# audioku/meta-transfer-learning

Measured on AMD Instinct MI355X. Metric: meta-steps/sec, higher is better.
Workload: dtype f32 (emulated: 3x3 conv + input Linear on 2 x fp16 pieces "h2" = 22 significand bits, big GEMMs and attention (d_k = 64) on 3 x bf16 pieces "x3" = exact fp32 operands, small products on fp32 MFMA, element-wise on VALU; fp32 accumulation everywhere)

## Files before the change

meta-transfer-learning_amd/csrc/mtl_mfma.hip:

```cpp
#include <cstdlib>
#include <type_traits>

#include "mtl_common.h"
#include "mtl_h2.h"
#include "../../include/mtl_hip.h"

namespace {

constexpr int BK = 32;
constexpr int NT = 256;

template <int ROWS>
struct LdsK {
    static constexpr int LD = BK + 1;
    static constexpr int SIZE = ROWS * LD;
    static __device__ __forceinline__ int at(int row, int k) { return row * LD + k; }
};
template <int ROWS>
struct LdsMN {
    static constexpr int LD = ROWS + 4;
    static constexpr int SIZE = BK * LD;
    static __device__ __forceinline__ int at(int row, int k) { return k * LD + row; }
};

// ... 534 lines not shown
struct EpiConvDgrad {
    float* dx;
    const float* act;
    int b, t0, f0, T, F, Cout, n0;
    __device__ __forceinline__ void store4(int lr, int lc, const float (&v)[4]) const {
        const int col = n0 + lc;
        const int w = (lr >> 5) * 8 + ((lr >> 2) & 7);
#pragma unroll
        for (int j = 0; j < 4; ++j) {
            const int t = t0 + 2 * (w >> 3) + (j & 1), f = f0 + 2 * (w & 7) + (j >> 1);
            if (t < T && f < F) {
                const long o = (((long)b * T + t) * F + f) * Cout + col;
                dx[o] = act[o] > 0.f ? v[j] : 0.f;
            }
        }
    }
    __device__ __forceinline__ void gate4(int lr, int lc, float (&m)[4]) const {
        const int col = n0 + lc;
        const int w = (lr >> 5) * 8 + ((lr >> 2) & 7);
#pragma unroll
        for (int j = 0; j < 4; ++j) {
            const int t = min(t0 + 2 * (w >> 3) + (j & 1), T - 1), f = min(f0 + 2 * (w & 7) + (j >> 1), F - 1);
            m[j] = __builtin_nontemporal_load(act + (((long)b * T + t) * F + f) * Cout + col);
        }
    }
    __device__ __forceinline__ void store4g(int lr, int lc, const float (&v)[4], const float (&m)[4]) const {
        const int col = n0 + lc;
        const int w = (lr >> 5) * 8 + ((lr >> 2) & 7);
#pragma unroll
        for (int j = 0; j < 4; ++j) {
            const int t = t0 + 2 * (w >> 3) + (j & 1), f = f0 + 2 * (w & 7) + (j >> 1);
            if (t < T && f < F) __builtin_nontemporal_store(m[j] > 0.f ? v[j] : 0.f, dx + (((long)b * T + t) * F + f) * Cout + col);
        }
    }
    __device__ __forceinline__ void gate4x2(int lr, int lc, f32x2v (&m)[4]) const {
        const int col = n0 + lc;
        const int w = (lr >> 5) * 8 + ((lr >> 2) & 7);
#pragma unroll
        for (int j = 0; j < 4; ++j) {
            const int t = min(t0 + 2 * (w >> 3) + (j & 1), T - 1), f = min(f0 + 2 * (w & 7) + (j >> 1), F - 1);
            m[j] = __builtin_nontemporal_load(reinterpret_cast<const f32x2v*>(act + (((long)b * T + t) * F + f) * Cout + col));
        }
    }
    __device__ __forceinline__ void store4x2g(int lr, int lc, const float (&v0)[4], const float (&v1)[4], const f32x2v (&m)[4]) const {
        const int col = n0 + lc;
        const int w = (lr >> 5) * 8 + ((lr >> 2) & 7);
#pragma unroll
        for (int j = 0; j < 4; ++j) {
            const int t = t0 + 2 * (w >> 3) + (j & 1), f = f0 + 2 * (w & 7) + (j >> 1);
            const f32x2v o = {m[j].x > 0.f ? v0[j] : 0.f, m[j].y > 0.f ? v1[j] : 0.f};
            if (t < T && f < F) __builtin_nontemporal_store(o, reinterpret_cast<f32x2v*>(dx + (((long)b * T + t) * F + f) * Cout + col));
        }
    }
};

struct ConvP {
    const float* x;
    const uint8_t* am_in;
    const float* w;
    const float* bias;
    const float* act;
    float* y;
    uint8_t* am_out;
    ConvGeom g;
    int ntile;
};

enum { EPI_RELU = 0, EPI_POOL = 1, EPI_DGRAD = 2 };

template <int BN, bool UNPOOL, int EPI>
__global__ __launch_bounds__(NT) void conv3x3_kernel(ConvP p) {
    using LA = LoadConvA<UNPOOL>;
    using LB = LoadMNMajor<BN, true>;
    using E = Engine<128, BN, LA, LB>;
    extern __shared__ __attribute__((aligned(16))) float smem[];
    const int tid = threadIdx.x;
    const int b = blockIdx.z / p.ntile, n0 = (blockIdx.z % p.ntile) * BN;
    const int t0 = blockIdx.y * 8, f0 = blockIdx.x * 16;
    LA la;
    LB lb;
    la.init(p.x, p.am_in, p.g, p.g.Cin, b, t0, f0, tid);
    lb.init(p.w, p.g.Cout, n0, p.g.Cout, 9 * p.g.Cin, tid);
    f32x16 acc[E::TM][E::TN];
    E::zero(acc);
    E::run(la, lb, 9 * p.g.Cin / BK, smem, acc);
    if (EPI == EPI_RELU) {
        EpiConvRelu e{p.y, p.bias, b, t0, f0, p.g.T, p.g.F, p.g.Cout, n0};
        E::finish(acc, e);
    } else if (EPI == EPI_POOL) {
        EpiConvPool e{p.y, p.am_out, p.bias, b, t0, f0, p.g.Tp, p.g.Fp, p.g.Cout, n0};
        E::finish(acc, e);
    } else {
        EpiConvDgrad e{p.y, p.act, b, t0, f0, p.g.T, p.g.F, p.g.Cout, n0};
        E::finish(acc, e);
    }
}

template <int BN, bool UNPOOL, int EPI>
int launch_conv(const ConvP& p, int Te, int Fe, hipStream_t s) {
    using E = Engine<128, BN, LoadConvA<UNPOOL>, LoadMNMajor<BN, true>>;
    static int attr = set_smem(conv3x3_kernel<BN, UNPOOL, EPI>, E::SMEM_BYTES);
    if (attr) return attr;
    dim3 grid((Fe + 15) / 16, (Te + 7) / 8, p.g.B * p.ntile);
    hipLaunchKernelGGL((conv3x3_kernel<BN, UNPOOL, EPI>), grid, dim3(NT), E::SMEM_BYTES, s, p);
    MTL_CHECK_LAUNCH();
    return MTL_OK;
}

template <bool UNPOOL, int EPI>
int dispatch_conv(ConvP& p, int Te, int Fe, hipStream_t s) {
    if (p.g.Cin % 32 || p.g.Cout % 64) return MTL_EINVAL;
    if (p.g.Cout % 128 == 0) {
        p.ntile = p.g.Cout / 128;
        return launch_conv<128, UNPOOL, EPI>(p, Te, Fe, s);
    }
    p.ntile = p.g.Cout / 64;
    return launch_conv<64, UNPOOL, EPI>(p, Te, Fe, s);
}

typedef __bf16 bf16x8 __attribute__((ext_vector_type(8)));
typedef __bf16 bf16x4 __attribute__((ext_vector_type(4)));
constexpr int X3_ROWB = 80;

__device__ __forceinline__ void split3(float x, __bf16& h, __bf16& m, __bf16& l) {
    h = (__bf16)x;
    const float r = x - (float)h;
    m = (__bf16)r;
    l = (__bf16)(r - (float)m);
}

typedef __bf16 bf16x2 __attribute__((ext_vector_type(2)));
__device__ __forceinline__ void split3x2(float x0, float x1, unsigned& h, unsigned& m, unsigned& l) {
    h = __builtin_bit_cast(unsigned, __builtin_convertvector(f32x2{x0, x1}, bf16x2));
    const float r0 = x0 - __builtin_bit_cast(float, h << 16), r1 = x1 - __builtin_bit_cast(float, h & 0xffff0000u);
    m = __builtin_bit_cast(unsigned, __builtin_convertvector(f32x2{r0, r1}, bf16x2));
    const float q0 = r0 - __builtin_bit_cast(float, m << 16), q1 = r1 - __builtin_bit_cast(float, m & 0xffff0000u);
    l = __builtin_bit_cast(unsigned, __builtin_convertvector(f32x2{q0, q1}, bf16x2));
}
__device__ __forceinline__ void split3x4(const float4& v, bf16x4& h, bf16x4& m, bf16x4& l) {
    uint2 hh, mm, ll;
    split3x2(v.x, v.y, hh.x, mm.x, ll.x);
    split3x2(v.z, v.w, hh.y, mm.y, ll.y);
    h = __builtin_bit_cast(bf16x4, hh);
    m = __builtin_bit_cast(bf16x4, mm);
    l = __builtin_bit_cast(bf16x4, ll);
}

typedef float f32x4 __attribute__((ext_vector_type(4)));
#ifndef X3H_IH
#define X3H_IH 0
#endif
#ifndef X3H_M16
#define X3H_M16 1
#endif
template <int NP>
struct Split;
template <>
struct Split<3> {
    static __device__ __forceinline__ void x2(float x0, float x1, float, unsigned (&pc)[3]) { split3x2(x0, x1, pc[0], pc[1], pc[2]); }
    static __device__ __forceinline__ f32x16 mfma(const uint4 (&a)[3], const uint4 (&b)[3], f32x16 cc) {
        const bf16x8 a0 = __builtin_bit_cast(bf16x8, a[0]), a1 = __builtin_bit_cast(bf16x8, a[1]), a2 = __builtin_bit_cast(bf16x8, a[2]);
        const bf16x8 b0 = __builtin_bit_cast(bf16x8, b[0]), b1 = __builtin_bit_cast(bf16x8, b[1]), b2 = __builtin_bit_cast(bf16x8, b[2]);
        cc = __builtin_amdgcn_mfma_f32_32x32x16_bf16(a2, b0, cc, 0, 0, 0);
        cc = __builtin_amdgcn_mfma_f32_32x32x16_bf16(a1, b1, cc, 0, 0, 0);
        cc = __builtin_amdgcn_mfma_f32_32x32x16_bf16(a0, b2, cc, 0, 0, 0);
        cc = __builtin_amdgcn_mfma_f32_32x32x16_bf16(a1, b0, cc, 0, 0, 0);
        cc = __builtin_amdgcn_mfma_f32_32x32x16_bf16(a0, b1, cc, 0, 0, 0);
        return __builtin_amdgcn_mfma_f32_32x32x16_bf16(a0, b0, cc, 0, 0, 0);
    }
    static __device__ __forceinline__ f32x4 mfma16(const uint4 (&a)[3], const uint4 (&b)[3], f32x4 cc) {
        const bf16x8 a0 = __builtin_bit_cast(bf16x8, a[0]), a1 = __builtin_bit_cast(bf16x8, a[1]), a2 = __builtin_bit_cast(bf16x8, a[2]);
        const bf16x8 b0 = __builtin_bit_cast(bf16x8, b[0]), b1 = __builtin_bit_cast(bf16x8, b[1]), b2 = __builtin_bit_cast(bf16x8, b[2]);
        cc = __builtin_amdgcn_mfma_f32_16x16x32_bf16(a2, b0, cc, 0, 0, 0);
        cc = __builtin_amdgcn_mfma_f32_16x16x32_bf16(a1, b1, cc, 0, 0, 0);
        cc = __builtin_amdgcn_mfma_f32_16x16x32_bf16(a0, b2, cc, 0, 0, 0);
        cc = __builtin_amdgcn_mfma_f32_16x16x32_bf16(a1, b0, cc, 0, 0, 0);
        cc = __builtin_amdgcn_mfma_f32_16x16x32_bf16(a0, b1, cc, 0, 0, 0);
        return __builtin_amdgcn_mfma_f32_16x16x32_bf16(a0, b0, cc, 0, 0, 0);
    }
};
template <>
struct Split<2> {
    static __device__ __forceinline__ void x2(float x0, float x1, float s, unsigned (&pc)[2]) { split2x2(x0 * s, x1 * s, pc[0], pc[1]); }
    static __device__ __forceinline__ f32x16 mfma(const uint4 (&a)[2], const uint4 (&b)[2], f32x16 cc) { return h2_mfma(a, b, cc); }
    static __device__ __forceinline__ f32x4 mfma16(const uint4 (&a)[2], const uint4 (&b)[2], f32x4 cc) {
        const f16x8 a0 = __builtin_bit_cast(f16x8, a[0]), a1 = __builtin_bit_cast(f16x8, a[1]);
        const f16x8 b0 = __builtin_bit_cast(f16x8, b[0]), b1 = __builtin_bit_cast(f16x8, b[1]);
        cc = __builtin_amdgcn_mfma_f32_16x16x32_f16(a1, b0, cc, 0, 0, 0);
        cc = __builtin_amdgcn_mfma_f32_16x16x32_f16(a0, b1, cc, 0, 0, 0);
        return __builtin_amdgcn_mfma_f32_16x16x32_f16(a0, b0, cc, 0, 0, 0);
    }
};
template <int NP>
__device__ __forceinline__ void split_x4(const float4& v, float s, uint2 (&pc)[NP]) {
    unsigned a[NP], b[NP];
    Split<NP>::x2(v.x, v.y, s, a);
    Split<NP>::x2(v.z, v.w, s, b);
#pragma unroll
    for (int q = 0; q < NP; ++q) pc[q] = make_uint2(a[q], b[q]);
}


constexpr int WSCALE_PARTS = 16;
template <int NP>
__global__ void conv_wprep_x3_kernel(const float* w, unsigned short* wf, unsigned short* wd, int Cout, int Cin) {
    const int total = 9 * Cin * Cout;
    const int nkf = 9 * (Cin / 32), nkd = 9 * (Cout / 32);
    float s = 1.f;
    if (NP == 2) {
        float* hf = reinterpret_cast<float*>(wf + (long)NP * total);
        float mx = 0.f;
#pragma unroll
        for (int i = 1; i <= WSCALE_PARTS; ++i) mx = fmaxf(mx, hf[i]);
        s = pow2_scale(mx);
        if (blockIdx.x == 0 && threadIdx.x == 0) {
            hf[0] = s;
            *reinterpret_cast<float*>(wd + (long)NP * total) = s;
        }
    }
    for (int e = blockIdx.x * blockDim.x + threadIdx.x; e < total; e += gridDim.x * blockDim.x) {
        const int tap = e % 9;
        const int cin = (e / 9) % Cin;
        const int cout = e / (9 * Cin);
        unsigned pc[NP];
        Split<NP>::x2(w[e], 0.f, s, pc);
#pragma unroll
        for (int p = 0; p < NP; ++p) {
            const unsigned short v = (unsigned short)(pc[p] & 0xffffu);
            wf[(((long)p * nkf + tap * (Cin / 32) + (cin >> 5)) * Cout + cout) * 32 + x3_swz(cin & 31, cout)] = v;
            wd[(((long)p * nkd + (8 - tap) * (Cout / 32) + (cout >> 5)) * Cin + cin) * 32 + x3_swz(cout & 31, cin)] = v;
        }
    }
}

__global__ __launch_bounds__(256) void conv_wscale_kernel(const float* w, int total, float* hdr_f) {
    __shared__ float sh[4];
    float mx = 0.f;
    for (int e = (blockIdx.x * 256 + threadIdx.x) * 4; e < total; e += WSCALE_PARTS * 1024) {
        const float4 v = *reinterpret_cast<const float4*>(w + e);
        mx = fmaxf(fmaxf(mx, fmaxf(fabsf(v.x), fabsf(v.y))), fmaxf(fabsf(v.z), fabsf(v.w)));
    }
    mx = wave_max(mx);
    if ((threadIdx.x & 63) == 0) sh[threadIdx.x >> 6] = mx;
    __syncthreads();
    if (threadIdx.x == 0) hdr_f[1 + blockIdx.x] = fmaxf(fmaxf(sh[0], sh[1]), fmaxf(sh[2], sh[3]));
}

struct ConvX3P {
    const float* x;
    const uint8_t* am_in;
    const unsigned char* w3;
    const float* bias;
    const float* act;
    float* y;
    uint8_t* am_out;
    ConvGeom g;
    int ntile;
    int dbg;
    int ntf, ntt, tiles;
    const float* amax_in;
    float* amax_out;
    int Bt;
    long sW, sBias, sAmaxIn, sAmaxOut;
    const int* widths;
    int wshift;
#ifdef MTL_X3_PROF
    unsigned long long* prof;
#endif
};
#ifdef MTL_X3_PROF
static unsigned long long* g_x3_prof = nullptr;
extern "C" void mtl_x3_prof_set(void* buf) { g_x3_prof = (unsigned long long*)buf; }
#define X3_T(v) const unsigned long long v = __builtin_amdgcn_s_memtime()
#define X3_ACC(slot, a, b) prof_acc[slot] += (b) - (a)
#define X3_PROF_DECL unsigned long long prof_acc[8] = {0, 0, 0, 0, 0, 0, 0, 0}
#define X3_PROF_FLUSH()                                                                                    \
    if (p.prof && (threadIdx.x & 63) == 0) {                                                               \
        for (int k_ = 0; k_ < 8; ++k_) p.prof[((long)blockIdx.x * 16 + (threadIdx.x >> 6)) * 8 + k_] = prof_acc[k_]; \
    }
#else
#define X3_T(v)
#define X3_ACC(slot, a, b)
#define X3_PROF_DECL
#define X3_PROF_FLUSH()
#endif

constexpr int XH_HF = 18;

struct X3Tile {
    int b, n0, t0, f0;
};

inline int device_cu_count() {
    int dev = 0, n = 0;
    if (hipGetDevice(&dev) != hipSuccess || hipDeviceGetAttribute(&n, hipDeviceAttributeMultiprocessorCount, dev) != hipSuccess || n <= 0)
        n = 256;
    return n;
}

template <int G>
__device__ inline int x3_task_rows(const ConvX3P& p, int task) {
    const int r = ((p.widths[task] >> p.wshift) + 8 * G - 1) / (8 * G);
    return r < p.ntt ? (r < 1 ? 1 : r) : p.ntt;
}

template <int G>
__device__ inline int x3_total_tiles(const ConvX3P& p) {
    if (!p.widths) return p.tiles;
    const int nt = p.g.B / p.Bt;
    int total = 0;
    for (int k = 0; k < nt; ++k) total += p.Bt * p.ntile * x3_task_rows<G>(p, k) * p.ntf;
    return total;
}

struct X3Cur {
    int k = 0, lo = 0, hi = -1, ntt = 0;
};

template <int G>
__device__ inline X3Tile x3_tile(const ConvX3P& p, int id, X3Cur& c) {
    X3Tile t;
    int ntt = p.ntt, b0 = 0;
    if (p.widths) {
        const int per_row = p.Bt * p.ntile * p.ntf, nt = p.g.B / p.Bt;
        if (c.hi < 0 || id < c.lo) {
            c.k = 0;
            c.lo = 0;
            c.ntt = x3_task_rows<G>(p, 0);
            c.hi = per_row * c.ntt;
        }
        while (id >= c.hi && c.k < nt - 1) {
            ++c.k;
            c.lo = c.hi;
            c.ntt = x3_task_rows<G>(p, c.k);
            c.hi = c.lo + per_row * c.ntt;
        }
        id -= c.lo;
        ntt = c.ntt;
        b0 = c.k * p.Bt;
    }
    const int fx = id % p.ntf;
    id /= p.ntf;
    const int ty = id % ntt;
    id /= ntt;
    t.f0 = fx * 16;
    t.t0 = ty * (8 * G);
    t.n0 = id % p.ntile;
    t.b = b0 + id / p.ntile;
    return t;
}

template <int BN, int G, bool UNPOOL, int EPI, int NP, int WN>
__global__ __launch_bounds__((2 * WN * G + 4) * 64) __attribute__((amdgpu_waves_per_eu(WN == 1 ? 4 : 1)))
void conv3x3_x3h_kernel(ConvX3P p) {
    constexpr int CW = 2 * WN;
    constexpr int WTM = 64, WTN = BN / WN, TM = WTM / 32, TN = WTN / 32;
    constexpr int XH_HT = 8 * G + 2, XH_NPIX = XH_HT * XH_HF;
    constexpr int XH_APLANE = XH_NPIX * X3_ROWB;
    constexpr int NHALO = 3 * 64;
    constexpr int XH_NVA = (XH_NPIX * 8 + NHALO - 1) / NHALO;
    constexpr int NCONS = CW * G * 64;
    constexpr int BPLANE = BN * 64, BBUF = NP * BPLANE, ABUF = NP * XH_APLANE;
    constexpr int NDMA = BBUF / 1024;
    extern __shared__ __attribute__((aligned(16))) unsigned char smx[];
    unsigned char* smA = smx;
    unsigned char* smB = smx + ABUF;
    const int tid = threadIdx.x;
    const int Cin = p.g.Cin, Cout = p.g.Cout, cch = Cin / BK, nk = 9 * cch;
    const int T = p.g.T, F = p.g.F, Tp = p.g.Tp, Fp = p.g.Fp;
    const int my_tiles = (x3_total_tiles<G>(p) - (int)blockIdx.x + (int)gridDim.x - 1) / (int)gridDim.x;
    if (my_tiles <= 0) return;
    const int nstage = my_tiles * cch;
    const int nstep = nstage * 9;

    if (tid >= NCONS + 64) {
        const int ptid = tid - NCONS - 64;
        float sx = NP == 2 ? pow2_scale(amax_read(p.amax_in)) : 1.f;
        int sx_task = 0;
        X3Cur cur_scale, cur_halo;
        auto set_scale = [&](int qc) {
            if (NP != 2 || p.Bt >= p.g.B) return;
            const int tk = x3_tile<G>(p, blockIdx.x + (qc / cch) * gridDim.x, cur_scale).b / p.Bt;
            if (tk != sx_task) {
                sx_task = tk;
                sx = pow2_scale(amax_read(p.amax_in + tk * p.sAmaxIn));
            }
        };
        float4 hv[XH_NVA];
        uchar4 ha[XH_NVA];
        unsigned hm[XH_NVA];
        auto fetch_halo = [&](int q) {
            const int j = q / cch, c = q - j * cch;
            const X3Tile tl = x3_tile<G>(p, blockIdx.x + j * gridDim.x, cur_halo);
#pragma unroll
            for (int i = 0; i < XH_NVA; ++i) {
                const int e = ptid + i * NHALO;
                const int hp = min(e >> 3, XH_NPIX - 1), c4 = (e & 7) * 4;
                const int ht = hp / XH_HF, hf = hp - ht * XH_HF;
                const int ts = tl.t0 + ht - 1, fs = tl.f0 + hf - 1;
                bool ok = (e >> 3) < XH_NPIX && (unsigned)ts < (unsigned)T && (unsigned)fs < (unsigned)F;
                const int tc = min(max(ts, 0), T - 1), fc = min(max(fs, 0), F - 1);
                if (!UNPOOL) {
                    hv[i] = *reinterpret_cast<const float4*>(p.x + (((long)tl.b * T + tc) * F + fc) * Cin + c * BK + c4);
                    hm[i] = ok ? 1u : 0u;
                } else {
                    const int tp = tc >> 1, fp = fc >> 1;
                    ok = ok && tp < Tp && fp < Fp;
                    const long o = (((long)tl.b * Tp + min(tp, Tp - 1)) * Fp + min(fp, Fp - 1)) * Cin + c * BK + c4;
                    ha[i] = *reinterpret_cast<const uchar4*>(p.am_in + o);
                    hv[i] = *reinterpret_cast<const float4*>(p.x + o);
                    hm[i] = (ok ? 1u : 0u) | ((unsigned)(((fs & 1) << 1) | (ts & 1)) << 1);
                }
            }
        };
        auto commit_halo = [&]() {
#pragma unroll
            for (int i = 0; i < XH_NVA; ++i) {
                const int e = ptid + i * NHALO;
                if ((e >> 3) >= XH_NPIX) continue;
                float4 v = hv[i];
                const bool ok = hm[i] & 1u;
                if (!UNPOOL) {
                    v = mask4(v, ok ? 15u : 0u);
                } else {
                    const unsigned sub = hm[i] >> 1;
                    v.x = (ok && ha[i].x == sub) ? v.x : 0.f;
                    v.y = (ok && ha[i].y == sub) ? v.y : 0.f;
                    v.z = (ok && ha[i].z == sub) ? v.z : 0.f;
                    v.w = (ok && ha[i].w == sub) ? v.w : 0.f;
                }
                uint2 pc[NP];
                split_x4<NP>(v, sx, pc);
                unsigned char* dst = smA + (e >> 3) * X3_ROWB + (e & 7) * 8;
#pragma unroll
                for (int q = 0; q < NP; ++q) *reinterpret_cast<uint2*>(dst + q * XH_APLANE) = pc[q];
            }
        };
        const bool doA = !(p.dbg & 2);
        X3_PROF_DECL;
        X3_T(h0);
        if (doA) fetch_halo(0);
        set_scale(0);
        if (doA) commit_halo();
        if (nstage > 1 && doA) fetch_halo(1);
        __syncthreads();
        X3_T(h1);
        X3_ACC(0, h0, h1);
#pragma unroll 1
        for (int q = 0; q < nstage; ++q) {
            X3_T(a0);
#pragma unroll 1
            for (int tap = 0; tap < 9; ++tap) __syncthreads();
            X3_T(a1);
            X3_ACC(1, a0, a1);
            if (q + 1 < nstage) {
                set_scale(q + 1);
                if (doA) commit_halo();
                X3_T(a2);
                X3_ACC(2, a1, a2);
                if (q + 2 < nstage && doA) fetch_halo(q + 2);
                X3_T(a3);
                X3_ACC(3, a2, a3);
                __syncthreads();
                X3_T(a4);
                X3_ACC(4, a3, a4);
            }
        }
        X3_PROF_FLUSH();
        return;
    }
    if (tid >= NCONS) {
        const int lane = tid & 63;
        const bool doB = !(p.dbg & 4);
        int dma_j = -1, dma_n0 = 0;
        X3Cur cur_dma;
        const unsigned char* dma_w3 = p.w3;
        auto dma = [&](int s_) {
            const int q = s_ / 9, tap = s_ - q * 9;
            const int j = q / cch, c = q - j * cch;
            if (j != dma_j && (p.ntile != 1 || p.Bt < p.g.B)) {
                const X3Tile tl = x3_tile<G>(p, blockIdx.x + j * gridDim.x, cur_dma);
                dma_n0 = tl.n0 * BN;
                dma_w3 = p.w3 + (tl.b / p.Bt) * p.sW;
                dma_j = j;
            }
            const int n0 = dma_n0;
            const unsigned char* w3 = dma_w3;
            const int kt = tap * cch + c;
            unsigned char* dst = smB + (s_ % 3) * BBUF;
#pragma unroll
            for (int i = 0; i < NDMA; ++i) {
                const int piece = i / (BN / 16), r16 = i - piece * (BN / 16);
                const unsigned char* g = w3 + (((long)piece * nk + kt) * Cout + n0 + r16 * 16) * 64 + lane * 16;
                __builtin_amdgcn_global_load_lds((const __attribute__((address_space(1))) void*)g,
                                                 (__attribute__((address_space(3))) void*)(dst + i * 1024), 16, 0, 0);
            }
        };
        if (doB) {
            dma(0);
            if (nstep > 1) dma(1);
        }
        if (nstep > 1) asm volatile("s_waitcnt vmcnt(%0)" ::"n"(NDMA) : "memory");
        else asm volatile("s_waitcnt vmcnt(0)" ::: "memory");
        __builtin_amdgcn_s_barrier();
        int tap = 0, q = 0;
        X3_PROF_DECL;
#pragma unroll 1
        for (int s_ = 0; s_ < nstep; ++s_) {
            X3_T(w0);
            if (s_ + 2 < nstep) {
                if (doB) dma(s_ + 2);
                X3_T(w1);
                X3_ACC(0, w0, w1);
                asm volatile("s_waitcnt vmcnt(%0)" ::"n"(NDMA) : "memory");
                X3_T(w2);
                X3_ACC(1, w1, w2);
            } else {
                asm volatile("s_waitcnt vmcnt(0)" ::: "memory");
            }
            X3_T(w3);
            __builtin_amdgcn_s_barrier();
            X3_T(w4);
            X3_ACC(2, w3, w4);
            if (++tap == 9) {
                tap = 0;
                if (++q < nstage) __builtin_amdgcn_s_barrier();
                X3_T(w5);
                X3_ACC(3, w4, w5);
            }
        }
        X3_PROF_FLUSH();
        return;
    }

    const int lane = tid & 63, wave = tid >> 6;
    const int grp = wave / CW, w4 = wave % CW;
    const int wm = w4 / WN, wn = w4 % WN, l31 = lane & 31, hi = lane >> 5;
    constexpr bool M16 = X3H_M16 != 0 && !(BN == 64 && G == 2 && WN == 2 && EPI == EPI_DGRAD && !UNPOOL);
    constexpr int TM16 = WTM / 16, TN16 = WTN / 16;
    f32x16 acc[M16 ? 1 : TM][M16 ? 1 : TN];
    f32x4 acc4[M16 ? TM16 : 1][M16 ? TN16 : 1];
    const int l15 = lane & 15, q4 = lane >> 4;
    float inv = 1.f, mx = 0.f;
    if (NP == 2) inv = 1.f / (pow2_scale(amax_read(p.amax_in)) * *reinterpret_cast<const float*>(p.w3 + (long)NP * nk * Cout * 64));
    int cur_task = 0;
    X3Cur cur_epi;
    const float* bias_t = p.bias;
    auto raise_bound = [&]() {
        if (!p.amax_out) return;
        float bmax = 0.f;
        if (EPI != EPI_DGRAD) {
            if (M16) {
#pragma unroll
                for (int jn = 0; jn < TN16; ++jn)
                    for (int nt = 0; nt < p.ntile; ++nt)
                        bmax = fmaxf(bmax, fabsf(bias_t[nt * BN + wn * WTN + (jn >> 1) * 32 + 2 * l15 + (jn & 1)]));
            } else
#pragma unroll
            for (int jn = 0; jn < TN; ++jn)
                for (int nt = 0; nt < p.ntile; ++nt) bmax = fmaxf(bmax, fabsf(bias_t[nt * BN + wn * WTN + jn * 32 + l31]));
        }
        amax_raise(p.amax_out + cur_task * p.sAmaxOut, mx + bmax);
    };
    int abase[TM];
#pragma unroll
    for (int i = 0; i < TM; ++i) {
        int t, f;
        tile_row_to_tf(wm * WTM + i * 32 + l31, t, f);
        abase[i] = ((t + grp * 8 + 1) * XH_HF + (f + 1)) * X3_ROWB + hi * 16;
#ifdef X3_FAKE_A
        abase[i] = (XH_HF + 1 + l31 + i * 32 + grp * 64) * X3_ROWB + hi * 16;
#endif
    }
    int abase16[M16 ? TM16 : 1];
    if (M16) {
#pragma unroll
        for (int i = 0; i < TM16; ++i) {
            int t, f;
            tile_row_to_tf(wm * WTM + i * 16 + l15, t, f);
            abase16[i] = ((t + grp * 8 + 1) * XH_HF + (f + 1)) * X3_ROWB + q4 * 16;
        }
    }
    const unsigned char* bBase16 = smB + (wn * WTN + 2 * l15) * 64 + ((q4 ^ ((l15 >> 1) & 3)) * 16);
    const unsigned char* bBase = smB + (wn * WTN + l31) * 64;
    int bsw[BK / 16];
#pragma unroll
    for (int st = 0; st < BK / 16; ++st) bsw[st] = (((st * 2 + hi) ^ ((l31 >> 2) & 3))) * 16;
    __syncthreads();
    int bst = 0;
    X3_PROF_DECL;
    X3_T(k0);
#pragma unroll 1
    for (int j = 0; j < my_tiles; ++j) {
        if (M16) {
#pragma unroll
            for (int i = 0; i < TM16; ++i)
#pragma unroll
                for (int jn = 0; jn < TN16; ++jn) acc4[i][jn] = f32x4{0.f, 0.f, 0.f, 0.f};
        } else {
#pragma unroll
            for (int i = 0; i < TM; ++i)
#pragma unroll
                for (int jn = 0; jn < TN; ++jn)
#pragma unroll
                    for (int v = 0; v < 16; ++v) acc[i][jn][v] = 0.f;
        }
#pragma unroll 1
        for (int c = 0; c < cch; ++c) {
#pragma unroll 1
            for (int tap = 0; tap < 9; ++tap, bst = bst == 2 ? 0 : bst + 1) {
                const int kh = tap / 3, kw = tap - kh * 3;
                const int toff = ((kw - 1) * XH_HF + (kh - 1)) * X3_ROWB;
                const unsigned char* bS = bBase + bst * BBUF;
                X3_T(c0);
                if (M16) {
                    const unsigned char* bS16 = bBase16 + bst * BBUF;
                    uint4 b16[TN16][NP];
#pragma unroll
                    for (int jn = 0; jn < TN16; ++jn)
#pragma unroll
                        for (int pc = 0; pc < NP; ++pc)
                            b16[jn][pc] = *reinterpret_cast<const uint4*>(bS16 + pc * BPLANE + ((jn >> 1) * 32 + (jn & 1)) * 64);
                    constexpr int IH = X3H_IH ? X3H_IH : 2;
#pragma unroll
                    for (int ih = 0; ih < TM16; ih += IH) {
                        uint4 a16[IH][NP];
#pragma unroll
                        for (int i = 0; i < IH; ++i)
#pragma unroll
                            for (int pc = 0; pc < NP; ++pc)
                                a16[i][pc] = *reinterpret_cast<const uint4*>(smA + pc * XH_APLANE + abase16[ih + i] + toff);
#pragma unroll
                        for (int i = 0; i < IH; ++i)
#pragma unroll
                            for (int jn = 0; jn < TN16; ++jn) acc4[ih + i][jn] = Split<NP>::mfma16(a16[i], b16[jn], acc4[ih + i][jn]);
                    }
                } else
#pragma unroll
                for (int st = 0; st < BK / 16; ++st) {
                    uint4 a[TM][NP], bb[TN][NP];
#pragma unroll
                    for (int i = 0; i < TM; ++i)
#pragma unroll
                        for (int pc = 0; pc < NP; ++pc)
                            a[i][pc] = *reinterpret_cast<const uint4*>(smA + pc * XH_APLANE + abase[i] + toff + st * 32);
#pragma unroll
                    for (int jn = 0; jn < TN; ++jn)
#pragma unroll
                        for (int pc = 0; pc < NP; ++pc)
                            bb[jn][pc] = *reinterpret_cast<const uint4*>(bS + pc * BPLANE + jn * 32 * 64 + bsw[st]);
#pragma unroll
                    for (int i = 0; i < TM; ++i)
#pragma unroll
                        for (int jn = 0; jn < TN; ++jn) acc[i][jn] = Split<NP>::mfma(a[i], bb[jn], acc[i][jn]);
                }
                X3_T(c1);
                X3_ACC(0, c0, c1);
                __syncthreads();
                X3_T(c2);
                X3_ACC(1, c1, c2);
            }
            X3_T(e0);
            if (c + 1 == cch && !(p.dbg & 8)) {
                int jj = j;
                asm volatile("" : "+s"(jj));
                const X3Tile tl = x3_tile<G>(p, blockIdx.x + jj * gridDim.x, cur_epi);
                const int ts0 = tl.t0 + grp * 8, n0 = tl.n0 * BN;
                if (p.Bt < p.g.B) {
                    const int tk = tl.b / p.Bt;
                    if (tk != cur_task) {
                        raise_bound();
                        mx = 0.f;
                        cur_task = tk;
                        bias_t = p.bias + tk * p.sBias;
                        if (NP == 2)
                            inv = 1.f / (pow2_scale(amax_read(p.amax_in + tk * p.sAmaxIn)) *
                                         *reinterpret_cast<const float*>(p.w3 + tk * p.sW + (long)NP * nk * Cout * 64));
                    }
                }
                auto walk = [&](auto&& epi) {
                    if (M16) {
#pragma unroll
                        for (int i = 0; i < TM16; ++i)
#pragma unroll
                            for (int jn = 0; jn < TN16; jn += 2) {
                                float v0[4], v1[4];
#pragma unroll
                                for (int k = 0; k < 4; ++k) {
                                    v0[k] = NP == 2 ? acc4[i][jn][k] * inv : acc4[i][jn][k];
                                    v1[k] = NP == 2 ? acc4[i][jn + 1][k] * inv : acc4[i][jn + 1][k];
                                    mx = fmaxf(mx, fmaxf(fabsf(v0[k]), fabsf(v1[k])));
                                }
                                epi.store4x2(wm * WTM + i * 16 + 4 * q4, wn * WTN + (jn >> 1) * 32 + 2 * l15, v0, v1);
                            }
                        return;
                    }
#pragma unroll
                    for (int i = 0; i < TM; ++i)
#pragma unroll
                        for (int jn = 0; jn < TN; ++jn)
#pragma unroll
                            for (int g = 0; g < 4; ++g) {
                                float v[4] = {acc[i][jn][4 * g], acc[i][jn][4 * g + 1], acc[i][jn][4 * g + 2], acc[i][jn][4 * g + 3]};
                                if (NP == 2) {
#pragma unroll
                                    for (int k = 0; k < 4; ++k) v[k] *= inv;
                                }
                                mx = fmaxf(fmaxf(mx, fmaxf(fabsf(v[0]), fabsf(v[1]))), fmaxf(fabsf(v[2]), fabsf(v[3])));
                                epi.store4(wm * WTM + i * 32 + 8 * g + 4 * hi, wn * WTN + jn * 32 + l31, v);
                            }
                };
                if (EPI == EPI_RELU) {
                    walk(EpiConvRelu{p.y, bias_t, tl.b, ts0, tl.f0, T, F, Cout, n0});
                } else if (EPI == EPI_POOL) {
                    walk(EpiConvPool{p.y, p.am_out, bias_t, tl.b, ts0, tl.f0, Tp, Fp, Cout, n0});
                } else {
                    const EpiConvDgrad epi{p.y, p.act, tl.b, ts0, tl.f0, T, F, Cout, n0};
                    if (M16) {
                        f32x2v gate16[TM16][TN16 / 2][4];
#pragma unroll
                        for (int i = 0; i < TM16; ++i)
#pragma unroll
                            for (int jp = 0; jp < TN16 / 2; ++jp) epi.gate4x2(wm * WTM + i * 16 + 4 * q4, wn * WTN + jp * 32 + 2 * l15, gate16[i][jp]);
#pragma unroll
                        for (int i = 0; i < TM16; ++i)
#pragma unroll
                            for (int jp = 0; jp < TN16 / 2; ++jp) {
                                float v0[4], v1[4];
#pragma unroll
                                for (int k = 0; k < 4; ++k) {
                                    v0[k] = NP == 2 ? acc4[i][2 * jp][k] * inv : acc4[i][2 * jp][k];
                                    v1[k] = NP == 2 ? acc4[i][2 * jp + 1][k] * inv : acc4[i][2 * jp + 1][k];
                                    mx = fmaxf(mx, fmaxf(fabsf(v0[k]), fabsf(v1[k])));
                                }
                                epi.store4x2g(wm * WTM + i * 16 + 4 * q4, wn * WTN + jp * 32 + 2 * l15, v0, v1, gate16[i][jp]);
                            }
                    } else {
                    float gate[TM][TN][4][4];
#pragma unroll
                    for (int i = 0; i < TM; ++i)
#pragma unroll
                        for (int jn = 0; jn < TN; ++jn)
#pragma unroll
                            for (int g = 0; g < 4; ++g)
                                epi.gate4(wm * WTM + i * 32 + 8 * g + 4 * hi, wn * WTN + jn * 32 + l31, gate[i][jn][g]);
#pragma unroll
                    for (int i = 0; i < TM; ++i)
#pragma unroll
                        for (int jn = 0; jn < TN; ++jn)
#pragma unroll
                            for (int g = 0; g < 4; ++g) {
                                float v[4] = {acc[i][jn][4 * g], acc[i][jn][4 * g + 1], acc[i][jn][4 * g + 2], acc[i][jn][4 * g + 3]};
                                if (NP == 2) {
#pragma unroll
                                    for (int k = 0; k < 4; ++k) v[k] *= inv;
                                }
                                mx = fmaxf(fmaxf(mx, fmaxf(fabsf(v[0]), fabsf(v[1]))), fmaxf(fabsf(v[2]), fabsf(v[3])));
                                epi.store4g(wm * WTM + i * 32 + 8 * g + 4 * hi, wn * WTN + jn * 32 + l31, v, gate[i][jn][g]);
                            }
                    }
                }
            }
            X3_T(e1);
            X3_ACC(2, e0, e1);
            if (j * cch + c + 1 < nstage) __syncthreads();
            X3_T(e2);
            X3_ACC(3, e1, e2);
        }
    }
    X3_T(k1);
    X3_ACC(4, k0, k1);
    X3_PROF_FLUSH();
    raise_bound();
}

template <int BN, int G, bool UNPOOL, int EPI, int NP, int WN = 2>
int launch_conv_x3h(ConvX3P p, int Te, int Fe, hipStream_t s) {
    constexpr int SMEM = NP * (8 * G + 2) * XH_HF * X3_ROWB + 3 * NP * BN * 64;
    constexpr int THREADS = (2 * WN * G + 4) * 64;
    static int attr = set_smem(conv3x3_x3h_kernel<BN, G, UNPOOL, EPI, NP, WN>, SMEM);
    if (attr) return attr;
    static const int per_cu = (THREADS <= 512 && SMEM <= 80 * 1024) ? 2 : 1;
    static const int ncu = device_cu_count();
    p.dbg = 0;
#ifdef MTL_X3_PROF
    p.prof = g_x3_prof;
#endif
    p.ntf = (Fe + 15) / 16;
    p.ntt = (Te + 8 * G - 1) / (8 * G);
    p.tiles = p.ntf * p.ntt * p.g.B * p.ntile;
    const int grid = p.tiles < ncu * per_cu ? p.tiles : ncu * per_cu;
    hipLaunchKernelGGL((conv3x3_x3h_kernel<BN, G, UNPOOL, EPI, NP, WN>), dim3(grid), dim3(THREADS), SMEM, s, p);
    MTL_CHECK_LAUNCH();
    return MTL_OK;
}

template <bool UNPOOL, int EPI, int NP>
int dispatch_conv_x3(ConvX3P& p, int Te, int Fe, hipStream_t s) {
    if (p.g.Cin % 64 || p.g.Cout % 64) return MTL_EINVAL;
    if (p.g.Cout % 128 == 0) {
        p.ntile = p.g.Cout / 128;
        return launch_conv_x3h<128, 2, UNPOOL, EPI, NP>(p, Te, Fe, s);
    }
    p.ntile = p.g.Cout / 64;
    if constexpr (NP == 2 && EPI != EPI_DGRAD) return launch_conv_x3h<64, 2, UNPOOL, EPI, NP, 1>(p, Te, Fe, s);
    if (p.g.Cin == 64) return launch_conv_x3h<64, 1, UNPOOL, EPI, NP>(p, Te, Fe, s);
    return launch_conv_x3h<64, 2, UNPOOL, EPI, NP>(p, Te, Fe, s);
}

struct WgradGeom {
    int B, T, F;
    int Ty, Fy;
    int Tp, Fp;
    int Cin, Cout;
    long npix;
    long per_split;
};

struct PixCursor {
    int b, t, f;
    __device__ __forceinline__ void set(long pix, int Ty, int Fy) {
        const int plane = Ty * Fy;
        b = (int)(pix / plane);
        const int rem = (int)(pix - (long)b * plane);
        t = rem / Fy;
        f = rem - t * Fy;
    }
    __device__ __forceinline__ void advance(int n, int Ty, int Fy) {
        f += n;
        while (f >= Fy) {
            f -= Fy;
            if (++t >= Ty) {
                t = 0;
                ++b;
            }
        }
    }
};

template <int ROWS>
struct LoadWgradX {
    using Lds = LdsMN<ROWS>;
    static constexpr int VPR = ROWS / 4, KPP = NT / VPR, NV = BK / KPP;
    struct Regs {
        float4 v[NV];
        unsigned m[NV];
    };
    const float* x;
    WgradGeom g;
    int dt, df, cofs, m4, k0;
    bool row_ok;
    long pbeg, pend;
    PixCursor cur[NV];
    __device__ void init(const float* x_, const WgradGeom& g_, int m0, long pbeg_, long pend_, int tid) {
        x = x_;
        g = g_;
        m4 = (tid % VPR) * 4;
        k0 = tid / VPR;
        const int m = m0 + m4;
        row_ok = m < 9 * g.Cin;
        const int tap = row_ok ? m / g.Cin : 0;
        cofs = row_ok ? m - tap * g.Cin : 0;
        const int kh = tap / 3, kw = tap - kh * 3;
        dt = kw - 1;
        df = kh - 1;
        pbeg = pbeg_;
        pend = pend_;
#pragma unroll
        for (int i = 0; i < NV; ++i) cur[i].set(min(pbeg + k0 + i * KPP, g.npix - 1), g.Ty, g.Fy);
    }
    __device__ __forceinline__ void fetch(int kt, Regs& r, int) {
#pragma unroll
        for (int i = 0; i < NV; ++i) {
            const long pix = pbeg + (long)kt * BK + k0 + i * KPP;
            bool ok = row_ok && pix < pend;
            const int ts = cur[i].t + dt, fs = cur[i].f + df;
            ok = ok && (unsigned)ts < (unsigned)g.T && (unsigned)fs < (unsigned)g.F;
            const int tc = min(max(ts, 0), g.T - 1), fc = min(max(fs, 0), g.F - 1);
            const int bc = min(cur[i].b, g.B - 1);
            r.v[i] = *reinterpret_cast<const float4*>(x + (((long)bc * g.T + tc) * g.F + fc) * g.Cin + cofs);
            r.m[i] = ok ? 15u : 0u;
            cur[i].advance(BK, g.Ty, g.Fy);
        }
    }
    __device__ __forceinline__ void commit(float* lds, const Regs& r, int) const {
#pragma unroll
        for (int i = 0; i < NV; ++i)
            *reinterpret_cast<float4*>(&lds[(k0 + i * KPP) * Lds::LD + m4]) = mask4(r.v[i], r.m[i]);
    }
};

template <int BN, bool UNPOOL>
struct LoadWgradDy {
    using Lds = LdsMN<BN>;
    static constexpr int VPR = BN / 4, KPP = NT / VPR, NV = BK / KPP;
    struct Regs {
        float4 v[NV];
        uchar4 a[NV];
        unsigned m[NV];
    };
    const float* dy;
    const uint8_t* am;
    WgradGeom g;
    int n0, m4, k0;
    long pbeg, pend;
    PixCursor cur[NV];
    __device__ void init(const float* dy_, const uint8_t* am_, const WgradGeom& g_, int n0_, long pbeg_, long pend_, int tid) {
        dy = dy_;
        am = am_;
        g = g_;
        n0 = n0_;
        m4 = (tid % VPR) * 4;
        k0 = tid / VPR;
        pbeg = pbeg_;
        pend = pend_;
        if (UNPOOL) {
#pragma unroll
            for (int i = 0; i < NV; ++i) cur[i].set(min(pbeg + k0 + i * KPP, g.npix - 1), g.Ty, g.Fy);
        }
    }
    __device__ __forceinline__ void fetch(int kt, Regs& r, int) {
#pragma unroll
        for (int i = 0; i < NV; ++i) {
            const long pix = pbeg + (long)kt * BK + k0 + i * KPP;
            const bool ok = pix < pend;
            if (!UNPOOL) {
                r.v[i] = *reinterpret_cast<const float4*>(dy + (ok ? pix : pbeg) * g.Cout + n0 + m4);
                r.m[i] = ok ? 1u : 0u;
            } else {
                const int t = cur[i].t, f = cur[i].f, bc = min(cur[i].b, g.B - 1);
                const long o = (((long)bc * g.Tp + (t >> 1)) * g.Fp + (f >> 1)) * g.Cout + n0 + m4;
                r.a[i] = *reinterpret_cast<const uchar4*>(am + o);
                r.v[i] = *reinterpret_cast<const float4*>(dy + o);
                r.m[i] = (ok ? 1u : 0u) | ((unsigned)(((f & 1) << 1) | (t & 1)) << 1);
                cur[i].advance(BK, g.Ty, g.Fy);
            }
        }
    }
    __device__ __forceinline__ void commit(float* lds, const Regs& r, int) const {
#pragma unroll
        for (int i = 0; i < NV; ++i) {
            float4 v = r.v[i];
            const bool ok = r.m[i] & 1u;
            if (!UNPOOL) {
                v = mask4(v, ok ? 15u : 0u);
            } else {
                const unsigned sub = r.m[i] >> 1;
                v.x = (ok && r.a[i].x == sub) ? v.x : 0.f;
                v.y = (ok && r.a[i].y == sub) ? v.y : 0.f;
                v.z = (ok && r.a[i].z == sub) ? v.z : 0.f;
                v.w = (ok && r.a[i].w == sub) ? v.w : 0.f;
            }
            *reinterpret_cast<float4*>(&lds[(k0 + i * KPP) * Lds::LD + m4]) = v;
        }
    }
};

struct EpiPartial {
// ... 1204 lines not shown
```

Baseline: 19.30.

## Route 64-wide fp16 dgrad convs to slim single-wave-N kernel variant

Sends Cout%128!=0 dgrad conv cases on the 2-piece fp16 path to the WN=1 kernel configuration (G=2), which allows four waves per EU. It also adds a register-slim specialization for that variant: halo masks are packed into one bitmask, unpool sub-positions are recomputed instead of stored, and addressing uses scalar bases with 32-bit offsets. A dedicated gated-ReLU epilogue prefetches gate values in batches and uses nontemporal loads and stores. Wave max reductions switch to ds_swizzle plus readlane. The intent is higher occupancy and less VGPR pressure, at the cost of less N-parallelism per block and added code complexity.

```diff
diff --git a/meta-transfer-learning_amd/csrc/mtl_mfma.hip b/meta-transfer-learning_amd/csrc/mtl_mfma.hip
--- a/meta-transfer-learning_amd/csrc/mtl_mfma.hip
+++ b/meta-transfer-learning_amd/csrc/mtl_mfma.hip
@@ -710,6 +710,12 @@
 #endif
 #ifndef X3H_M16
 #define X3H_M16 1
+#endif
+#ifndef X3H_DG2
+#define X3H_DG2 1
+#endif
+#ifndef X3H_DG5
+#define X3H_DG5 1
 #endif
 template <int NP>
 struct Split;
@@ -908,9 +914,34 @@
     return t;
 }
 
+template <bool SWZ>
+__device__ __forceinline__ float x3_wave_max(float v) {
+    if constexpr (!SWZ) {
+        return wave_max(v);
+    } else {
+        v = fmaxf(v, __int_as_float(__builtin_amdgcn_ds_swizzle(__float_as_int(v), (1 << 10) | 0x1f)));
+        v = fmaxf(v, __int_as_float(__builtin_amdgcn_ds_swizzle(__float_as_int(v), (2 << 10) | 0x1f)));
+        v = fmaxf(v, __int_as_float(__builtin_amdgcn_ds_swizzle(__float_as_int(v), (4 << 10) | 0x1f)));
+        v = fmaxf(v, __int_as_float(__builtin_amdgcn_ds_swizzle(__float_as_int(v), (8 << 10) | 0x1f)));
+        v = fmaxf(v, __int_as_float(__builtin_amdgcn_ds_swizzle(__float_as_int(v), (16 << 10) | 0x1f)));
+        return fmaxf(__int_as_float(__builtin_amdgcn_readlane(__float_as_int(v), 0)), __int_as_float(__builtin_amdgcn_readlane(__float_as_int(v), 32)));
+    }
+}
+template <bool SWZ>
+__device__ __forceinline__ float x3_amax_read(const float* a) {
+    return x3_wave_max<SWZ>(a[(threadIdx.x & (MTL_AMAX_SLOTS - 1)) * MTL_AMAX_STRIDE]);
+}
+template <bool SWZ>
+__device__ __forceinline__ void x3_amax_raise(float* a, float mx) {
+    mx = x3_wave_max<SWZ>(mx);
+    float* slot = a + (blockIdx.x & (MTL_AMAX_SLOTS - 1)) * MTL_AMAX_STRIDE;
+    if ((threadIdx.x & 63) == 0 && mx > *slot) atomicMax(reinterpret_cast<unsigned*>(slot), __float_as_uint(mx));
+}
+
 template <int BN, int G, bool UNPOOL, int EPI, int NP, int WN>
 __global__ __launch_bounds__((2 * WN * G + 4) * 64) __attribute__((amdgpu_waves_per_eu(WN == 1 ? 4 : 1)))
 void conv3x3_x3h_kernel(ConvX3P p) {
+    constexpr bool SLIM = WN == 1 && EPI == EPI_DGRAD;
     constexpr int CW = 2 * WN;
     constexpr int WTM = 64, WTN = BN / WN, TM = WTM / 32, TN = WTN / 32;
     constexpr int XH_HT = 8 * G + 2, XH_NPIX = XH_HT * XH_HF;
@@ -933,7 +964,7 @@
 
     if (tid >= NCONS + 64) {
         const int ptid = tid - NCONS - 64;
-        float sx = NP == 2 ? pow2_scale(amax_read(p.amax_in)) : 1.f;
+        float sx = NP == 2 ? pow2_scale(x3_amax_read<SLIM>(p.amax_in)) : 1.f;
         int sx_task = 0;
         X3Cur cur_scale, cur_halo;
         auto set_scale = [&](int qc) {
@@ -941,18 +972,20 @@
             const int tk = x3_tile<G>(p, blockIdx.x + (qc / cch) * gridDim.x, cur_scale).b / p.Bt;
             if (tk != sx_task) {
                 sx_task = tk;
-                sx = pow2_scale(amax_read(p.amax_in + tk * p.sAmaxIn));
+                sx = pow2_scale(x3_amax_read<SLIM>(p.amax_in + tk * p.sAmaxIn));
             }
         };
         float4 hv[XH_NVA];
         uchar4 ha[XH_NVA];
-        unsigned hm[XH_NVA];
+        unsigned hm[SLIM ? 1 : XH_NVA];
         auto fetch_halo = [&](int q) {
             const int j = q / cch, c = q - j * cch;
             const X3Tile tl = x3_tile<G>(p, blockIdx.x + j * gridDim.x, cur_halo);
+            int pt = ptid;
+            if constexpr (SLIM) asm volatile("" : "+v"(pt));
 #pragma unroll
             for (int i = 0; i < XH_NVA; ++i) {
-                const int e = ptid + i * NHALO;
+                const int e = pt + i * NHALO;
                 const int hp = min(e >> 3, XH_NPIX - 1), c4 = (e & 7) * 4;
                 const int ht = hp / XH_HF, hf = hp - ht * XH_HF;
                 const int ts = tl.t0 + ht - 1, fs = tl.f0 + hf - 1;
@@ -960,28 +993,40 @@
                 const int tc = min(max(ts, 0), T - 1), fc = min(max(fs, 0), F - 1);
                 if (!UNPOOL) {
                     hv[i] = *reinterpret_cast<const float4*>(p.x + (((long)tl.b * T + tc) * F + fc) * Cin + c * BK + c4);
-                    hm[i] = ok ? 1u : 0u;
+                    if constexpr (SLIM) hm[0] = i ? hm[0] | ((ok ? 1u : 0u) << i) : (ok ? 1u : 0u);
+                    else hm[i] = ok ? 1u : 0u;
                 } else {
                     const int tp = tc >> 1, fp = fc >> 1;
                     ok = ok && tp < Tp && fp < Fp;
+                    if constexpr (SLIM) {
+                        const long sbase = (long)__builtin_amdgcn_readfirstlane(tl.b) * Tp * Fp * Cin + c * BK;
+                        const unsigned o = (unsigned)((min(tp, Tp - 1) * Fp + min(fp, Fp - 1)) * Cin + c4);
+                        ha[i] = *reinterpret_cast<const uchar4*>(p.am_in + sbase + o);
+                        hv[i] = *reinterpret_cast<const float4*>(reinterpret_cast<const char*>(p.x + sbase) + o * 4u);
+                    } else {
                     const long o = (((long)tl.b * Tp + min(tp, Tp - 1)) * Fp + min(fp, Fp - 1)) * Cin + c * BK + c4;
                     ha[i] = *reinterpret_cast<const uchar4*>(p.am_in + o);
                     hv[i] = *reinterpret_cast<const float4*>(p.x + o);
-                    hm[i] = (ok ? 1u : 0u) | ((unsigned)(((fs & 1) << 1) | (ts & 1)) << 1);
+                    }
+                    if constexpr (SLIM) hm[0] = i ? hm[0] | ((ok ? 1u : 0u) << i) : (ok ? 1u : 0u);
+                    else hm[i] = (ok ? 1u : 0u) | ((unsigned)(((fs & 1) << 1) | (ts & 1)) << 1);
                 }
             }
         };
         auto commit_halo = [&]() {
+            int pt = ptid;
+            if constexpr (SLIM) asm volatile("" : "+v"(pt));
 #pragma unroll
             for (int i = 0; i < XH_NVA; ++i) {
-                const int e = ptid + i * NHALO;
+                const int e = pt + i * NHALO;
                 if ((e >> 3) >= XH_NPIX) continue;
                 float4 v = hv[i];
-                const bool ok = hm[i] & 1u;
+                const bool ok = SLIM ? (hm[0] >> i) & 1u : hm[i] & 1u;
                 if (!UNPOOL) {
                     v = mask4(v, ok ? 15u : 0u);
                 } else {
-                    const unsigned sub = hm[i] >> 1;
+                    const int ht_ = (e >> 3) / XH_HF, hf_ = (e >> 3) - ht_ * XH_HF;
+                    const unsigned sub = SLIM ? (unsigned)((((hf_ + 1) & 1) << 1) | ((ht_ + 1) & 1)) : hm[SLIM ? 0 : i] >> 1;
                     v.x = (ok && ha[i].x == sub) ? v.x : 0.f;
                     v.y = (ok && ha[i].y == sub) ? v.y : 0.f;
                     v.z = (ok && ha[i].z == sub) ? v.z : 0.f;
@@ -1094,13 +1139,14 @@
     const int lane = tid & 63, wave = tid >> 6;
     const int grp = wave / CW, w4 = wave % CW;
     const int wm = w4 / WN, wn = w4 % WN, l31 = lane & 31, hi = lane >> 5;
-    constexpr bool M16 = X3H_M16 != 0 && !(BN == 64 && G == 2 && WN == 2 && EPI == EPI_DGRAD && !UNPOOL);
+    constexpr bool M16 = X3H_M16 != 0 && !(BN == 64 && G == 2 && (WN == 2 || X3H_DG5 != 2) && EPI == EPI_DGRAD && !UNPOOL);
     constexpr int TM16 = WTM / 16, TN16 = WTN / 16;
+    constexpr int DGB16 = 2, DGB32 = 1;
     f32x16 acc[M16 ? 1 : TM][M16 ? 1 : TN];
     f32x4 acc4[M16 ? TM16 : 1][M16 ? TN16 : 1];
     const int l15 = lane & 15, q4 = lane >> 4;
     float inv = 1.f, mx = 0.f;
-    if (NP == 2) inv = 1.f / (pow2_scale(amax_read(p.amax_in)) * *reinterpret_cast<const float*>(p.w3 + (long)NP * nk * Cout * 64));
+    if (NP == 2) inv = 1.f / (pow2_scale(x3_amax_read<SLIM>(p.amax_in)) * *reinterpret_cast<const float*>(p.w3 + (long)NP * nk * Cout * 64));
     int cur_task = 0;
     X3Cur cur_epi;
     const float* bias_t = p.bias;
@@ -1118,7 +1164,7 @@
             for (int jn = 0; jn < TN; ++jn)
                 for (int nt = 0; nt < p.ntile; ++nt) bmax = fmaxf(bmax, fabsf(bias_t[nt * BN + wn * WTN + jn * 32 + l31]));
         }
-        amax_raise(p.amax_out + cur_task * p.sAmaxOut, mx + bmax);
+        x3_amax_raise<SLIM>(p.amax_out + cur_task * p.sAmaxOut, mx + bmax);
     };
     int abase[TM];
 #pragma unroll
@@ -1232,7 +1278,7 @@
                         cur_task = tk;
                         bias_t = p.bias + tk * p.sBias;
                         if (NP == 2)
-                            inv = 1.f / (pow2_scale(amax_read(p.amax_in + tk * p.sAmaxIn)) *
+                            inv = 1.f / (pow2_scale(x3_amax_read<SLIM>(p.amax_in + tk * p.sAmaxIn)) *
                                          *reinterpret_cast<const float*>(p.w3 + tk * p.sW + (long)NP * nk * Cout * 64));
                     }
                 }
@@ -1272,6 +1318,102 @@
                     walk(EpiConvRelu{p.y, bias_t, tl.b, ts0, tl.f0, T, F, Cout, n0});
                 } else if (EPI == EPI_POOL) {
                     walk(EpiConvPool{p.y, p.am_out, bias_t, tl.b, ts0, tl.f0, Tp, Fp, Cout, n0});
+                } else if constexpr (WN == 1 && EPI == EPI_DGRAD) {
+                    int el;
+                    asm volatile("v_mbcnt_lo_u32_b32 %0, -1, 0\n\tv_mbcnt_hi_u32_b32 %0, -1, %0" : "=v"(el));
+                    const int sb = __builtin_amdgcn_readfirstlane(tl.b), sf0 = __builtin_amdgcn_readfirstlane(tl.f0);
+                    const int st0 = __builtin_amdgcn_readfirstlane(ts0 + 4 * wm), sn0 = __builtin_amdgcn_readfirstlane(n0);
+                    auto gate_base = [&](int t, int cb) {
+                        return reinterpret_cast<const char*>(p.act + ((((long)sb * T + min(t, T - 1)) * F + sf0) * Cout + sn0 + cb));
+                    };
+                    auto out_base = [&](int t, int fu, int cb) {
+                        return reinterpret_cast<char*>(p.y + ((((long)sb * T + t) * F + sf0 + fu) * Cout + sn0 + cb));
+                    };
+                    if constexpr (M16) {
+                        constexpr int NG = TM16 * (TN16 / 2);
+                        constexpr int GB = DGB16, NB = NG / GB;
+                        static_assert(NG % GB == 0, "whole batches");
+                        const int fl = 2 * (el >> 4);
+                        const unsigned lcol = 2 * (el & 15);
+                        const unsigned so = (unsigned)(fl * Cout + lcol) * 4u;
+                        f32x2v gate16[NB > 1 ? 2 : 1][GB][4];
+                        auto load_gates = [&](int bt) {
+#pragma unroll
+                            for (int e = 0; e < GB; ++e) {
+                                const int u = bt * GB + e, i = u / (TN16 / 2), jp = u % (TN16 / 2);
+#pragma unroll
+                                for (int k = 0; k < 4; ++k) {
+                                    const int fc = min(sf0 + 8 * (i & 1) + (k >> 1) + fl, F - 1) - sf0;
+                                    gate16[bt & 1][e][k] = __builtin_nontemporal_load(reinterpret_cast<const f32x2v*>(
+                                        gate_base(st0 + 2 * (i >> 1) + (k & 1), jp * 32) + (unsigned)(fc * Cout + lcol) * 4u));
+                                }
+                            }
+                        };
+                        load_gates(0);
+#pragma unroll
+                        for (int bt = 0; bt < NB; ++bt) {
+                            if (bt + 1 < NB) load_gates(bt + 1);
+#pragma unroll
+                            for (int e = 0; e < GB; ++e) {
+                                const int u = bt * GB + e, i = u / (TN16 / 2), jp = u % (TN16 / 2);
+#pragma unroll
+                                for (int k = 0; k < 4; ++k) {
+                                    const float v0 = NP == 2 ? acc4[i][2 * jp][k] * inv : acc4[i][2 * jp][k];
+                                    const float v1 = NP == 2 ? acc4[i][2 * jp + 1][k] * inv : acc4[i][2 * jp + 1][k];
+                                    mx = fmaxf(mx, fmaxf(fabsf(v0), fabsf(v1)));
+                                    asm volatile("" : "+v"(mx));
+                                    const int t = st0 + 2 * (i >> 1) + (k & 1), fu = 8 * (i & 1) + (k >> 1);
+                                    const f32x2v m = gate16[bt & 1][e][k];
+                                    const f32x2v o = {m.x > 0.f ? v0 : 0.f, m.y > 0.f ? v1 : 0.f};
+                                    if (t < T && sf0 + fu + fl < F)
+                                        __builtin_nontemporal_store(o, reinterpret_cast<f32x2v*>(out_base(t, fu, jp * 32) + so));
+                                }
+                            }
+                        }
+                    } else {
+                        constexpr int NG = TM * TN * 4;
+                        constexpr int GB = DGB32, NB = NG / GB;
+                        static_assert(NG % GB == 0, "whole batches");
+                        const int fl = 2 * (el >> 5);
+                        const unsigned lcol = el & 31;
+                        const unsigned so = (unsigned)(fl * Cout + lcol) * 4u;
+                        float gate[NB > 1 ? 2 : 1][GB][4];
+                        auto load_gates = [&](int bt) {
+#pragma unroll
+                            for (int e = 0; e < GB; ++e) {
+                                const int u = bt * GB + e, i = u / (TN * 4), jn = (u >> 2) % TN, g = u & 3;
+#pragma unroll
+                                for (int k = 0; k < 4; ++k) {
+                                    const int fc = min(sf0 + 4 * g + (k >> 1) + fl, F - 1) - sf0;
+                                    gate[bt & 1][e][k] = __builtin_nontemporal_load(reinterpret_cast<const float*>(
+                                        gate_base(st0 + 2 * i + (k & 1), jn * 32) + (unsigned)(fc * Cout + lcol) * 4u));
+                                }
+                            }
+                        };
+                        load_gates(0);
+#pragma unroll
+                        for (int bt = 0; bt < NB; ++bt) {
+                            if (bt + 1 < NB) load_gates(bt + 1);
+#pragma unroll
+                            for (int e = 0; e < GB; ++e) {
+                                const int u = bt * GB + e, i = u / (TN * 4), jn = (u >> 2) % TN, g = u & 3;
+                                float v[4] = {acc[i][jn][4 * g], acc[i][jn][4 * g + 1], acc[i][jn][4 * g + 2], acc[i][jn][4 * g + 3]};
+                                if (NP == 2) {
+#pragma unroll
+                                    for (int k = 0; k < 4; ++k) v[k] *= inv;
+                                }
+                                mx = fmaxf(fmaxf(mx, fmaxf(fabsf(v[0]), fabsf(v[1]))), fmaxf(fabsf(v[2]), fabsf(v[3])));
+                                asm volatile("" : "+v"(mx));
+#pragma unroll
+                                for (int k = 0; k < 4; ++k) {
+                                    const int t = st0 + 2 * i + (k & 1), fu = 4 * g + (k >> 1);
+                                    if (t < T && sf0 + fu + fl < F)
+                                        __builtin_nontemporal_store(gate[bt & 1][e][k] > 0.f ? v[k] : 0.f,
+                                                                    reinterpret_cast<float*>(out_base(t, fu, jn * 32) + so));
+                                }
+                            }
+                        }
+                    }
                 } else {
                     const EpiConvDgrad epi{p.y, p.act, tl.b, ts0, tl.f0, T, F, Cout, n0};
                     if (M16) {
@@ -1362,6 +1504,12 @@
     }
     p.ntile = p.g.Cout / 64;
     if constexpr (NP == 2 && EPI != EPI_DGRAD) return launch_conv_x3h<64, 2, UNPOOL, EPI, NP, 1>(p, Te, Fe, s);
+    if constexpr (NP == 2 && UNPOOL && X3H_DG2 != 0) {
+        if (p.g.Cin == 64 && (long)p.g.Tp * p.g.Fp * p.g.Cin < (1L << 30)) return launch_conv_x3h<64, 2, UNPOOL, EPI, NP, 1>(p, Te, Fe, s);
+    }
+    if constexpr (NP == 2 && !UNPOOL && X3H_DG5 != 0) {
+        if (p.g.Cin != 64) return launch_conv_x3h<64, 2, UNPOOL, EPI, NP, 1>(p, Te, Fe, s);
+    }
     if (p.g.Cin == 64) return launch_conv_x3h<64, 1, UNPOOL, EPI, NP>(p, Te, Fe, s);
     return launch_conv_x3h<64, 2, UNPOOL, EPI, NP>(p, Te, Fe, s);
 }
```

Result: faster. 19.59 (median of 6 runs) (+1.5%).
